# conservation-laws/ryujin

Hardware: AMD Instinct MI355X
Metric: MDoF-updates/s per Euler forward step; achieved HBM GB/s vs roofline (higher is better)
Workload: dtype f64; 1 GPU; 2D Euler Mach-3 forward-facing step, Q1, SSPRK33 stage sequence (BASELINE.json configs[1]); gridpoints_per_gpu=2498844, gridpoints_total=2498844, dofs_total=9995376, cells_per_unit=995, partition=x-slabs x1, equal gridpoint counts, develop_updates=600

## Files before the change

### include/ryujin_hip.h

```cpp
#ifndef RYUJIN_HIP_H
#define RYUJIN_HIP_H

#include <stddef.h>
#include <stdint.h>

#ifdef __cplusplus
extern "C" {
#endif

#define RYUJIN_OK 0
#define RYUJIN_WARN 1
#define RYUJIN_RESTART 2
#define RYUJIN_ERR_TAU (-1)
#define RYUJIN_ERR_ARG (-2)
#define RYUJIN_ERR_HIP (-3)
#define RYUJIN_ERR_COMM (-4)
#define RYUJIN_ERR_UNSUPPORTED (-5)

enum {
  RYUJIN_EQ_EULER = 0,
  RYUJIN_EQ_SHALLOW_WATER = 1,
  RYUJIN_EQ_EULER_AEOS = 2,
  RYUJIN_EQ_SCALAR_CONSERVATION = 3
};
// ... 66 lines not shown
  int sc_use_greedy_wavespeed;
  int sc_use_averaged_entropy;
  int sc_random_entropies;

  int system_scope_events;
  int debug_join_exchanges;
  int debug_bc_fold_max_slices;
  int debug_no_small_mesh_split;
  int debug_pij_storage;
  int debug_expensive_bounds_check;
  int debug_tile_map;
  int debug_band_stride;
  int debug_xcd_chunk;
  int debug_stencil_classes;
  int debug_next_tile_mask;
} ryujin_hip_params;

typedef struct ryujin_hip_offline {
  uint32_t n_export, n_internal, n_owned, n_relevant;
  uint32_t simd_length;
  const uint64_t *row_starts;
  const uint32_t *columns;
  const double *cij;
  const double *mij;
  const double *mi;
  const double *mi_inv;
  double measure_of_omega;

  uint32_t n_bdry;
  const uint32_t *b_i;
// ... 87 lines not shown

int ryujin_hip_set_cfl(ryujin_hip_ctx *ctx, double cfl);
int ryujin_hip_get_cfl(ryujin_hip_ctx *ctx, double *cfl);
int ryujin_hip_set_id_violation_strategy(ryujin_hip_ctx *ctx, int strategy);
int ryujin_hip_get_alpha(ryujin_hip_ctx *ctx, double *alpha );
int ryujin_hip_get_counters(ryujin_hip_ctx *ctx, unsigned *n_restarts, unsigned *n_warnings);
int ryujin_hip_limiter_statistics(ryujin_hip_ctx *ctx, double *limited_slice_fraction, int *pij_stored,
                                  double *stored_slice_fraction);
int ryujin_hip_layout_info(ryujin_hip_ctx *ctx, unsigned long long *n_tiles, unsigned long long *n_regular_tiles);
int ryujin_hip_chain_info(ryujin_hip_ctx *ctx, unsigned long long *n_chained_tiles,
                          unsigned long long *n_chained_entries);
int ryujin_hip_stencil_class_info(ryujin_hip_ctx *ctx, unsigned long long *n_uniform_slices,
                                  unsigned long long *n_classes, double *uniform_entry_fraction);
int ryujin_hip_next_tile_mask_info(ryujin_hip_ctx *ctx, int *active, unsigned long long *n_tiles,
                                   unsigned long long *n_named);
int ryujin_hip_tile_statistics(ryujin_hip_ctx *ctx, double *stored_fraction, double *read_fraction,
                               double *formed_by_step6_fraction);

int ryujin_hip_debug_fetch(ryujin_hip_ctx *ctx, int what, double *out, size_t n_doubles);
int ryujin_hip_debug_fill(ryujin_hip_ctx *ctx, int what, double value);
#define RYUJIN_DEBUG_PLAN_LENGTH 32
int ryujin_hip_debug_plan(ryujin_hip_ctx *ctx, int *out, int n);
int ryujin_hip_set_timers(ryujin_hip_ctx *ctx, int enable);
int ryujin_hip_get_timers(ryujin_hip_ctx *ctx, double ms[8]);
int ryujin_hip_get_timers_accum(ryujin_hip_ctx *ctx, double ms[8], unsigned *n_updates, int reset);
int ryujin_hip_synchronize(ryujin_hip_ctx *ctx);
int ryujin_hip_event_record(ryujin_hip_ctx *ctx, int which );
int ryujin_hip_event_elapsed_ms(ryujin_hip_ctx *ctx, double *ms);
int ryujin_hip_debug_layout(const ryujin_hip_offline *offline, uint64_t *ptr, uint32_t *col,
                            uint64_t *transposed, const double *data, uint32_t n_comp, double *out);
// ... 156 lines not shown
```

### ryujin_amd/capi.py

```python
from __future__ import annotations

import ctypes as C
import os

import numpy as np

from . import _build

c_double_p = C.POINTER(C.c_double)
c_u32_p = C.POINTER(C.c_uint32)
c_u64_p = C.POINTER(C.c_uint64)
c_u8_p = C.POINTER(C.c_uint8)
c_int_p = C.POINTER(C.c_int)

RYUJIN_OK, RYUJIN_WARN, RYUJIN_RESTART = 0, 1, 2
RYUJIN_ERR_TAU, RYUJIN_ERR_ARG, RYUJIN_ERR_HIP, RYUJIN_ERR_COMM, RYUJIN_ERR_UNSUPPORTED = -1, -2, -3, -4, -5
EQ_EULER, EQ_SHALLOW_WATER, EQ_EULER_AEOS, EQ_SCALAR_CONSERVATION = 0, 1, 2, 3
FLUX_BURGERS, FLUX_KPP, FLUX_POLYNOMIAL, FLUX_FUNCTION = 0, 1, 2, 3
EOS_POLYTROPIC_GAS, EOS_NOBLE_ABEL_STIFFENED_GAS, EOS_VAN_DER_WAALS, EOS_JONES_WILKINS_LEE = 0, 1, 2, 3
EOS_FUNCTION = 4
EOS_PRESSURE, EOS_SPECIFIC_INTERNAL_ENERGY, EOS_TEMPERATURE, EOS_SPEED_OF_SOUND = 0, 1, 2, 3
BC_DO_NOTHING, BC_PERIODIC, BC_SLIP, BC_NO_SLIP, BC_DIRICHLET, BC_DYNAMIC, BC_DIRICHLET_MOMENTUM = range(7)
IDV_WARN, IDV_RAISE_EXCEPTION = 0, 1
CUT_NONE, CUT_BOX, CUT_CYLINDER = 0, 1, 2
# ... 30 lines not shown
        ("riemann_newton_max_iterations", C.c_int), ("riemann_newton_tolerance", C.c_double),
        ("eos", C.c_int), ("compute_strict_bounds", C.c_int),
        ("eos_covolume_b", C.c_double), ("eos_q", C.c_double), ("eos_pinf", C.c_double),
        ("eos_vdw_a", C.c_double), ("eos_gas_constant_R", C.c_double),
        ("jwl_A", C.c_double), ("jwl_B", C.c_double), ("jwl_R1", C.c_double), ("jwl_R2", C.c_double),
        ("jwl_omega", C.c_double), ("jwl_rho_0", C.c_double), ("jwl_q_0", C.c_double),
        ("jwl_cv", C.c_double),
        ("sc_flux", C.c_int), ("sc_flux_polynomial", (C.c_double * 4) * 3),
        ("sc_derivative_approximation_delta", C.c_double), ("sc_use_greedy_wavespeed", C.c_int),
        ("sc_use_averaged_entropy", C.c_int), ("sc_random_entropies", C.c_int),
        ("system_scope_events", C.c_int), ("debug_join_exchanges", C.c_int),
        ("debug_bc_fold_max_slices", C.c_int), ("debug_no_small_mesh_split", C.c_int),
        ("debug_pij_storage", C.c_int), ("debug_expensive_bounds_check", C.c_int),
        ("debug_tile_map", C.c_int), ("debug_band_stride", C.c_int),
        ("debug_xcd_chunk", C.c_int), ("debug_stencil_classes", C.c_int),
        ("debug_next_tile_mask", C.c_int),
    ]


class Offline(C.Structure):
    _fields_ = [
        ("n_export", C.c_uint32), ("n_internal", C.c_uint32), ("n_owned", C.c_uint32),
        ("n_relevant", C.c_uint32), ("simd_length", C.c_uint32),
        ("row_starts", c_u64_p), ("columns", c_u32_p), ("cij", c_double_p), ("mij", c_double_p),
        ("mi", c_double_p), ("mi_inv", c_double_p), ("measure_of_omega", C.c_double),
        ("n_bdry", C.c_uint32), ("b_i", c_u32_p), ("b_normal", c_double_p), ("b_id", c_u8_p),
        ("n_pairs", C.c_uint32), ("p_i", c_u32_p), ("p_col", c_u32_p), ("p_j", c_u32_p),
        ("initial_precomputed", c_double_p),
        ("n_nbr", C.c_int), ("nbr_rank", c_int_p), ("send_off", c_u32_p), ("send_idx", c_u32_p),
        ("recv_off", c_u32_p), ("row_send_off", c_u32_p), ("row_send_row", c_u32_p),
        ("row_send_col", c_u32_p),
# ... 336 lines not shown
        lib.ryujin_offline_file_positions.argtypes = [C.c_void_p]
        lib.ryujin_offline_file_b_positions.restype = c_double_p
        lib.ryujin_offline_file_b_positions.argtypes = [C.c_void_p]
        _synth = lib
    return _synth



HIP_SYMBOLS = [
    "ryujin_hip_comm_unique_id", "ryujin_hip_comm_init", "ryujin_hip_comm_init_local",
    "ryujin_hip_comm_init_loopback",
    "ryujin_hip_comm_destroy", "ryujin_hip_comm_info", "ryujin_hip_exchange_info", "ryujin_hip_device_count",
    "ryujin_hip_time_step_fn", "ryujin_hip_debug_addresses",
    "ryujin_hip_host_register", "ryujin_hip_host_unregister", "ryujin_hip_state_download_owned",
    "ryujin_hip_state_download_prepared", "ryujin_hip_layout_info", "ryujin_hip_chain_info", "ryujin_hip_stencil_class_info", "ryujin_hip_tile_statistics",
    "ryujin_hip_next_tile_mask_info", "ryujin_hip_debug_fill",
    "ryujin_hip_default_params", "ryujin_hip_create", "ryujin_hip_destroy",
    "ryujin_hip_state_alloc", "ryujin_hip_state_free", "ryujin_hip_state_upload",
    "ryujin_hip_state_download", "ryujin_hip_state_download_precomputed", "ryujin_hip_state_integrals",
    "ryujin_hip_prepare_state_vector", "ryujin_hip_step", "ryujin_hip_sadd", "ryujin_hip_time_step", "ryujin_hip_time_step_n",
    "ryujin_hip_get_timers_accum",
    "ryujin_hip_set_cfl", "ryujin_hip_get_cfl", "ryujin_hip_set_id_violation_strategy",
    "ryujin_hip_get_alpha", "ryujin_hip_get_counters", "ryujin_hip_limiter_statistics", "ryujin_hip_debug_fetch", "ryujin_hip_debug_plan",
    "ryujin_hip_set_timers", "ryujin_hip_get_timers", "ryujin_hip_synchronize",
    "ryujin_hip_event_record", "ryujin_hip_event_elapsed_ms", "ryujin_hip_last_error",
    "ryujin_hip_version", "ryujin_hip_debug_layout", "ryujin_hip_debug_pow", "ryujin_hip_debug_function", "ryujin_hip_debug_rk_outcome",
    "ryujin_hip_postprocess_configure", "ryujin_hip_postprocess_compute", "ryujin_hip_postprocess_download",
    "ryujin_hip_postprocess_bounds",
    "ryujin_hip_quantities_add_manifold", "ryujin_hip_quantities_reset", "ryujin_hip_quantities_clear_statistics",
    "ryujin_hip_quantities_accumulate", "ryujin_hip_quantities_instantaneous", "ryujin_hip_quantities_time_averaged",
    "ryujin_hip_quantities_time_series",
# ... 70 lines not shown
        lib.ryujin_hip_time_step_n.argtypes = [vp, C.c_int, C.c_int, C.c_int, c_int_p, c_double_p, C.c_double,
                                               C.c_int, C.c_double, C.c_double, c_double_p]
        lib.ryujin_hip_time_step_fn.argtypes = [vp, C.c_int, C.c_int, C.c_int, c_int_p, C.c_double, DIRICHLET_FN,
                                                C.c_void_p, C.c_double, C.c_int, C.c_double, C.c_double, c_double_p]
        lib.ryujin_hip_device_count.argtypes = [c_int_p]
        lib.ryujin_hip_layout_info.argtypes = [vp, C.POINTER(C.c_ulonglong), C.POINTER(C.c_ulonglong)]
        lib.ryujin_hip_chain_info.argtypes = [vp, C.POINTER(C.c_ulonglong), C.POINTER(C.c_ulonglong)]
        if hasattr(lib, "ryujin_hip_stencil_class_info"):
            lib.ryujin_hip_stencil_class_info.argtypes = [vp, C.POINTER(C.c_ulonglong), C.POINTER(C.c_ulonglong),
                                                          C.POINTER(C.c_double)]
        if hasattr(lib, "ryujin_hip_debug_fill"):
            lib.ryujin_hip_debug_fill.argtypes = [vp, C.c_int, C.c_double]
        if hasattr(lib, "ryujin_hip_next_tile_mask_info"):
            lib.ryujin_hip_next_tile_mask_info.argtypes = [vp, c_int_p, C.POINTER(C.c_ulonglong),
                                                           C.POINTER(C.c_ulonglong)]
        lib.ryujin_hip_tile_statistics.argtypes = [vp, C.POINTER(C.c_double), C.POINTER(C.c_double), C.POINTER(C.c_double)]
        lib.ryujin_hip_host_register.argtypes = [vp, C.c_void_p, C.c_size_t]
        lib.ryujin_hip_host_unregister.argtypes = [vp, C.c_void_p]
        lib.ryujin_hip_state_download_owned.argtypes = [vp, C.c_int, c_double_p]
        lib.ryujin_hip_state_download_prepared.argtypes = [vp, C.c_int, c_double_p]
        lib.ryujin_hip_debug_addresses.argtypes = [vp, c_u64_p]
        lib.ryujin_hip_debug_plan.argtypes = [vp, c_int_p, C.c_int]
        lib.ryujin_hip_synchronize.argtypes = [vp]
        lib.ryujin_hip_event_record.argtypes = [vp, C.c_int]
        lib.ryujin_hip_event_elapsed_ms.argtypes = [vp, c_double_p]
        lib.ryujin_hip_version.restype = C.c_char_p
        lib.ryujin_hip_debug_layout.argtypes = [C.POINTER(Offline), c_u64_p, c_u32_p, c_u64_p,
                                                c_double_p, C.c_uint32, c_double_p]
        lib.ryujin_hip_debug_pow.argtypes = [C.c_int, c_double_p, c_double_p, c_double_p, C.c_size_t]
        lib.ryujin_hip_debug_rk_outcome.argtypes = [C.c_int, C.c_int, C.c_int]
# ... 52 lines not shown
```

### ryujin_amd/csrc/host_context.hpp

```cpp

#pragma once

#include <algorithm>
#include <atomic>
#include <cmath>
#include <cstdint>
#include <cstring>
#include <numeric>
#include <stdexcept>
#include <string>
#include <vector>

#include "host_layout.hpp"
#include "ryujin_hip.h"

namespace ryujin_hip
{
  struct HipError : std::runtime_error {
    int status;
    HipError(int status, const std::string &what)
        : std::runtime_error(what)
        , status(status)
    {
    }
// ... 45 lines not shown
      if (p.eos < RYUJIN_EOS_POLYTROPIC_GAS || p.eos > RYUJIN_EOS_FUNCTION)
        throw HipError(RYUJIN_ERR_UNSUPPORTED, "unknown equation of state");
      for (uint32_t b = 0; b < o.n_bdry; ++b)
        if (o.b_id[b] == RYUJIN_BC_DYNAMIC)
          throw HipError(RYUJIN_ERR_UNSUPPORTED,
                         "euler aeos: dynamic boundary conditions are not implemented in the reference");
    }
    if (p.equation == RYUJIN_EQ_SHALLOW_WATER && p.dim == 3)
      throw HipError(RYUJIN_ERR_UNSUPPORTED, "the shallow water equations are defined for dim 1 and 2");
    if (p.dim < 1 || p.dim > 3)
      throw HipError(RYUJIN_ERR_ARG, "dim must be 1, 2 or 3");
    if (p.limiter_iterations < 0 || p.limiter_iterations > 2)
      throw HipError(RYUJIN_ERR_ARG, "The number of limiter iterations must be between [0,2]");
    if (p.debug_stencil_classes > 1)
      throw HipError(RYUJIN_ERR_ARG, "debug_stencil_classes must be < 0 (off), 0 or 1 (classes without the table of norms)");
    if (p.debug_pij_storage > 2)
      throw HipError(RYUJIN_ERR_ARG, "debug_pij_storage must be < 0, 0, 1 or 2 (per-tile P_ij in 3-D was retired)");
    if (p.equation == RYUJIN_EQ_SCALAR_CONSERVATION && p.sc_flux == RYUJIN_FLUX_FUNCTION &&
        (!(p.sc_derivative_approximation_delta > 0.) || !std::isfinite(p.sc_derivative_approximation_delta)))
      throw HipError(RYUJIN_ERR_ARG, "flux: derivative approximation delta must be positive and finite");
    if (o.discontinuous_ansatz != 0) {
      if (p.equation == RYUJIN_EQ_SCALAR_CONSERVATION)
        throw HipError(RYUJIN_ERR_UNSUPPORTED,
                       "discontinuous ansatz with scalar conservation equations: the reference's Riemann solver is 0/0 "
                       "on the structural zeros of a dG stencil");
      if (!o.incidence || !o.mass_matrix_inverse)
        throw HipError(RYUJIN_ERR_ARG, "discontinuous ansatz without incidence / inverse mass matrix");
    }
    if (o.n_nbr > 0 && !have_comm)
      throw HipError(RYUJIN_ERR_COMM, "offline data has neighbour ranks but no communicator was given");
// ... 166 lines not shown
```

### ryujin_amd/csrc/kernels_euler.hpp

```cpp

#pragma once

#include <hip/hip_runtime.h>

#include <cfloat>
#include <cstdint>

#include "euler_device.hpp"

namespace ryujin_hip
{
  struct DeviceScalars;

  struct StencilClassEntry {
    double c[2];
    double m;
    int32_t delta;
    uint32_t pad;
  };
  static_assert(sizeof(StencilClassEntry) == 32, "four 64-bit words");

  struct StepBegin {
    DeviceScalars *scalars;
    double tau_max_in, tau_in;
// ... 79 lines not shown
#endif
#ifndef RYUJIN_OCC_LAST_3D
#define RYUJIN_OCC_LAST_3D 4
#endif
#ifndef RYUJIN_LAST_CHUNK_3D
#define RYUJIN_LAST_CHUNK_3D 3
#endif
#ifndef RYUJIN_LAST_CHUNK_2D
#define RYUJIN_LAST_CHUNK_2D 3
#endif
#ifndef RYUJIN_OCC_DIJ
#define RYUJIN_OCC_DIJ 2
#endif
#ifndef RYUJIN_OCC_LOW
#define RYUJIN_OCC_LOW 3
#endif
#ifndef RYUJIN_OCC_LOW_AEOS
#define RYUJIN_OCC_LOW_AEOS 2
#endif
#ifndef RYUJIN_OCC_PIJ
#define RYUJIN_OCC_PIJ 2
#endif
#ifndef RYUJIN_OCC_HO
#define RYUJIN_OCC_HO 2
#endif
#ifndef RYUJIN_PER_SLICE_MAX_LIMITED
#define RYUJIN_PER_SLICE_MAX_LIMITED 0.8
#endif

  constexpr int kBlock = 256;
// ... 884 lines not shown
          d = dij[pos];
        }
        d_sum -= d;
      }
    }
    double tau = DBL_MAX;
    if (row_active) {
      d_sum = fmin(d_sum, -1.e6 * DBL_MIN);
      dij[(uint64_t)r.base * 64 + r.lane] = d_sum;
      tau = cfl * M.mi[i] / (-2. * d_sum);
    }
    publish_tau_min(scalars, wave_min(tau), r.lane);
  }

  template <int MAXW>
  __global__ void __launch_bounds__(kBlock)
  k_dij_diag_unrolled(const DeviceMesh M, const uint32_t *__restrict__ lower_mask, const double cfl,
                      double *__restrict__ dij, DeviceScalars *__restrict__ scalars)
  {
    const RowCtx r = row_context(M);
    if (!r.valid)
      return;
    const bool row_active = r.len > 1;
    uint32_t mask = row_active ? lower_mask[r.row] : 0u;
    asm volatile("" : "+v"(mask));
    double d[MAXW];
#pragma unroll
    for (int c = 1; c < MAXW; ++c) {
      d[c] = 0.;
      if ((uint32_t)c < r.width) {
        const uint32_t pos = (r.base + c) * 64 + r.lane;
        const TileDesc t = tile_desc<(MAXW <= 9)>(M, (uint64_t)r.base + c);
        const uint32_t src = ((mask >> c) & 1u) ? tile_transposed(M, t, (uint64_t)r.base + c, r.lane) : pos;
// ... 6 lines not shown
      if ((uint32_t)c < r.width) {
        if ((mask >> c) & 1u)
          dij[(r.base + c) * 64 + r.lane] = d[c];
        if (row_active && (uint32_t)c < r.len)
          d_sum -= d[c];
      }
    }
    double tau = DBL_MAX;
    if (row_active) {
      d_sum = fmin(d_sum, -1.e6 * DBL_MIN);
      dij[(uint64_t)r.base * 64 + r.lane] = d_sum;
      tau = cfl * M.mi[r.row] / (-2. * d_sum);
    }
    publish_tau_min(scalars, wave_min(tau), r.lane);
  }

  RYUJIN_DEV double finalize_tau(DeviceScalars *scalars)
  {
    const double tau_max = __longlong_as_double((long long)scalars->tau_max_bits);
    const int use_device_tau = scalars->use_device_tau;
    const double tau_in = scalars->tau_in;
    const double tau = use_device_tau ? scalars->tau_rk : (tau_in == 0. ? tau_max : tau_in);
    if (blockIdx.x == 0 && threadIdx.x == 0) {
      const int invalid = (isnan(tau_max) || isinf(tau_max) || !(tau_max > 0.)) ? 1 : 0;
      const int stage = scalars->stage;
      scalars->tau_invalid = invalid;
      if (invalid && scalars->tau_invalid_accum < kStageCode - stage)
        scalars->tau_invalid_accum = kStageCode - stage;
      scalars->tau = tau;
      if (!use_device_tau)
// ... 35 lines not shown
  {
    const double denom = fmax(d_ij, 100. * DBL_MIN);
    return 1. / denom;
  }

  template <bool DG>
  RYUJIN_DEV double high_order_factor(const double alpha_i, const double alpha_j, const double *incidence,
                                      const uint64_t pos)
  {
    double factor = (alpha_i + alpha_j) * .5;
    if constexpr (DG)
      factor = fmax(factor, incidence[pos]);
    return factor;
  }

  template <int DIM, bool HAS_STAGES, bool STORE_P = true, bool DG = false>
  __global__ void __launch_bounds__(kBlock, (DIM == 3 && HAS_STAGES) ? 1 : ((DIM == 3 || HAS_STAGES || DG) ? 2 : RYUJIN_OCC_LOW))
  k_low_order(const EulerParams P, const DeviceMesh M, DeviceScalars *scalars,
              const double weight, const StageArgs<DIM> S, const double *__restrict__ U,
              const double *__restrict__ prec, const double *__restrict__ alpha,
              const double *__restrict__ dij, double *__restrict__ new_U, double *__restrict__ r_out,
              double *__restrict__ bounds, double *__restrict__ pij)
  {
    using E = Euler<DIM>;
    constexpr int K = E::K;
    const RowCtx r = row_context(M);
    if (!r.valid)
      return;
    const bool row_active = r.len > 1;
    const uint32_t i = row_active ? r.row : (r.row < M.n_owned ? r.row : M.n_owned - 1);
    const double tau = finalize_tau(scalars);

    double U_i[K], U_i_new[K], F_iH[K];
    load_state<K>(U, i, U_i);
#pragma unroll
    for (int q = 0; q < K; ++q) {
      U_i_new[q] = U_i[q];
// ... 28 lines not shown
        if constexpr (UNIFORM)
          return (uint32_t)((int32_t)i + class_delta(M, cls + (uint32_t)(colbase - r.base)));
        else
          return ld_stream(cols + (colbase * 64 + r.lane));
      };
      uint32_t j_n = column(r.base);
      uint32_t j_nn = r.width > 1 ? column((uint64_t)r.base + 1) : i;
      double c_n[DIM], U_n[K];
      if constexpr (UNIFORM)
        class_cij<DIM>(M, cls, c_n);
      else
        load_entry<DIM>(cij, r.base, r.lane, c_n);
      double d_n = dij[(uint64_t)r.base * 64 + r.lane];
      load_state<K>(U, j_n, U_n);
      double alpha_n = alpha[j_n];
      double s_n = prec[(size_t)j_n * 2 + 0];

      for (uint32_t c = 0; c < r.width; ++c) {
        const uint64_t colbase = (uint64_t)r.base + c;
        const bool active = UNIFORM ? row_active : (row_active && c < r.len);
        double c_ij[DIM], U_j[K];
        const uint32_t j = j_n;
#pragma unroll
        for (int d = 0; d < DIM; ++d)
          c_ij[d] = c_n[d];
#pragma unroll
        for (int q = 0; q < K; ++q)
          U_j[q] = U_n[q];
        const double d_ij = d_n, alpha_j = alpha_n, s_j = s_n;
        if (c + 1 < r.width) {
          j_n = j_nn;
          if constexpr (UNIFORM)
            class_cij<DIM>(M, cls + c + 1, c_n);
          else
            load_entry<DIM>(cij, colbase + 1, r.lane, c_n);
          d_n = dij[(colbase + 1) * 64 + r.lane];
          load_state<K>(U, j_n, U_n);
          alpha_n = alpha[j_n];
          s_n = prec[(size_t)j_n * 2 + 0];
          j_nn = (c + 2 < r.width) ? column(colbase + 2) : i;
        }

        if (!active)
          continue;

        const double d_ijH = d_ij * high_order_factor<DG>(alpha_i, alpha_j, M.incidence, colbase * 64 + r.lane);
        double scaled_c_ij[DIM];
        const double inverse_denom = inverse_regularized(d_ij);
#pragma unroll
        for (int d = 0; d < DIM; ++d)
          scaled_c_ij[d] = c_ij[d] * inverse_denom;

        double f_j[K][DIM];
        E::flux(P, U_j, f_j);
// ... 25 lines not shown
          const double dU = U_j[q] - U_i[q];
          U_i_new[q] += tau * m_i_inv * d_ij * dU;
          F_iH[q] += d_ijH * dU;
          P_ij[q] += (d_ijH - d_ij) * dU;
        }

        {
          const double rho_i = U_i[0], rho_j = U_j[0];
          double dm_c = (U_i[1] - U_j[1]) * scaled_c_ij[0];
#pragma unroll
          for (int d = 1; d < DIM; ++d)
            dm_c += (U_i[1 + d] - U_j[1 + d]) * scaled_c_ij[d];
          const double rho_ij_bar = 0.5 * (rho_i + rho_j + dm_c) + 0.;
          rho_min = fmin(rho_min, rho_ij_bar);
          rho_max = fmax(rho_max, rho_ij_bar);
          s_min = fmin(s_min, s_j);
          rho_relaxation_numerator += 1. * (rho_i + rho_j);
          rho_relaxation_denominator += 1.;
          double U_avg[K];
#pragma unroll
          for (int q = 0; q < K; ++q)
            U_avg[q] = (U_i[q] + U_j[q]) * .5;
          const double s_interp = c == 0 ? s_j : E::specific_entropy(P, U_avg);
          s_interp_max = fmax(s_interp_max, s_interp);
        }

#pragma unroll
        for (int q = 0; q < K; ++q) {
          F_iH[q] += weight * flux_ij[q];
          P_ij[q] += weight * flux_ij[q];
        }

        if constexpr (HAS_STAGES) {
          for (int s = 0; s < S.stages; ++s) {
            double U_iHs[K], U_jHs[K];
            load_state<K>(S.U[s], i, U_iHs);
            load_state<K>(S.U[s], j, U_jHs);
            double f_iHs[K][DIM], f_jHs[K][DIM];
            E::flux(P, U_iHs, f_iHs);
// ... 16 lines not shown
    dispatch_uniform<kClasses>(cls, column_loop);

    if (!row_active)
      return;

    store_state<K>(new_U, i, U_i_new);
    store_state<K>(r_out, i, F_iH);

    const double hd_i = m_i * M.measure_of_omega_inverse;
    const double r_i = relaxation_radius<DIM>(hd_i) * P.lim_relaxation_factor;
    const double rho_relaxation =
        fabs(rho_relaxation_numerator) / (fabs(rho_relaxation_denominator) + DBL_EPSILON);
    const double relaxation = (2. * P.lim_relaxation_factor) * rho_relaxation;
    const double rho_min_r = fmax((1. - r_i) * rho_min, rho_min - relaxation);
    const double rho_max_r = fmin((1. + r_i) * rho_max, rho_max + relaxation);
    const double entropy_relaxation = P.lim_relaxation_factor * (s_interp_max - s_min);
    const double s_min_r = fmax((1. - r_i) * s_min, s_min - entropy_relaxation);

    const size_t stride = M.bounds_stride;
    bounds[i] = rho_min_r;
    bounds[stride + i] = rho_max_r;
    bounds[2 * stride + i] = s_min_r;
  }

  template <int NB, unsigned MAX_MASK>
  __global__ void __launch_bounds__(kBlock)
  k_bounds_combine_minmax(const DeviceMesh M, const double *__restrict__ in, double *__restrict__ out)
  {
    const RowCtx r = row_context(M);
    if (!r.valid)
      return;
    const bool row_active = r.len > 1;
    const uint32_t i = row_active ? r.row : (r.row < M.n_owned ? r.row : M.n_owned - 1);
    const size_t stride = M.bounds_stride;
    double b[NB];
#pragma unroll
    for (int q = 0; q < NB; ++q)
// ... 165 lines not shown
```

### ryujin_amd/csrc/ryujin_hip.hip

```cpp

#include <hip/hip_runtime.h>
#include <rccl/rccl.h>

#include <algorithm>
#include <atomic>
#include <cmath>
#include <cstddef>
#include <cstdlib>
#include <cstring>
#include <condition_variable>
#include <limits>
#include <memory>
#include <mutex>
#include <numeric>
#include <string>
#include <type_traits>
#include <vector>

#include "ryujin_hip.h"

#ifndef RYUJIN_XCD_CHUNK_3D
#define RYUJIN_XCD_CHUNK_3D 8
#endif

// ... 1274 lines not shown
{
  StepPlanInput in;
  in.equation = is_euler_v<E> ? PlanEquation::euler
                              : (is_aeos_v<E> ? PlanEquation::euler_aeos
                                              : (is_scalar_v<E> ? PlanEquation::scalar : PlanEquation::shallow_water));
  in.dim = E::DIMENSION;
  in.fusable_precompute = E::kFusablePrecompute;
  in.stages = stages;
  in.limiter_iterations = params.limiter_iterations;
  in.dg = dg;
  in.max_row_len = L.max_row_len;
  in.n_slices = L.n_slices;
  in.n_export_slices = exch.n_nbr != 0 ? n_export_slices : 0u;
  in.debug_pij_storage = params.debug_pij_storage;
  in.debug_next_tile_mask = params.debug_next_tile_mask;
  in.checked = params.debug_expensive_bounds_check != 0;
  in.limited_fraction = limited_fraction;
  in.per_slice_max_limited = (double)RYUJIN_PER_SLICE_MAX_LIMITED;
  in.resident_waves_step5 = resident_waves_step5;
  in.resident_waves_step6 = resident_waves_step6;
  in.bc_fold_max_slices = bc_fold_max_slices;
  in.pending_precompute = pending_precompute;
  in.riemann_newton_max_iterations = eparams.riemann_newton_max_iterations;
  in.rarefaction_power = eparams.rarefaction_power;
  in.friction = swparams.manning != 0.;
  return in;
}

template <typename E>
void ryujin_hip_ctx::step2_dij_alpha(const StepPlan &plan, const State &old)
// ... 71 lines not shown
      if (flux_interpreted_pairs())
        hipLaunchKernelGGL(k_dij_boundary_sc_function<DIM>, dim3(grid_for(n_pairs, kFluxFunctionBlock)),
                           dim3(kFluxFunctionBlock), 0, stream, eparams, d_flux_function.ptr, n_pairs, d_p_i.ptr,
                           d_p_j.ptr, d_p_pos.ptr, d_p_cji.ptr, old.U.ptr, old.prec.ptr, d_dij.ptr);
      else
        hipLaunchKernelGGL(k_dij_boundary_sc<DIM>, dim3(grid_for(n_pairs)), block, 0, stream, eparams,
                           n_pairs, d_p_i.ptr, d_p_j.ptr, d_p_pos.ptr, d_p_cji.ptr, old.U.ptr,
                           old.prec.ptr, d_dij.ptr);
    }
    else
      hipLaunchKernelGGL(k_dij_boundary<E>, dim3(grid_for(n_pairs)), block, 0, stream, eparams,
                         n_pairs, d_p_i.ptr, d_p_j.ptr, d_p_pos.ptr, d_p_cji.ptr, old.U.ptr, d_dij.ptr);
  }
  sweep([&](const DeviceMesh &mm, dim3 grid) {
    auto unrolled = [&](auto width) {
      hipLaunchKernelGGL(k_dij_diag_unrolled<decltype(width)::value>, grid, block, 0, launch_stream, mm,
                         d_lower_mask.ptr, params.cfl, d_dij.ptr, d_scalars.ptr);
    };
    if (plan.diag_width == 3)
      unrolled(std::integral_constant<int, 3>{});
    else if (plan.diag_width == 9)
      unrolled(std::integral_constant<int, 9>{});
    else if (plan.diag_width == 27)
      unrolled(std::integral_constant<int, 27>{});
    else
      hipLaunchKernelGGL(k_dij_diag, grid, block, 0, launch_stream, mm, params.cfl, d_dij.ptr,
                         d_scalars.ptr);
  });
  if (!(deferred && rk_stage > 0))
    allreduce_scalar(&d_scalars.ptr->tau_max_bits, 0);
  if (want_tau_early && deferred && rk_stage == 0) {
// ... 46 lines not shown
          });
        });
      }
    }
    auto launch4 = [&](auto has_stages, auto stores_p, auto dg_) {
      constexpr bool HS = decltype(has_stages)::value, SP = decltype(stores_p)::value, DG = decltype(dg_)::value;
      if constexpr (is_euler_v<E>)
        launch(k_low_order<DIM, HS, SP, DG>);
      else if constexpr (is_aeos_v<E>)
        launch(k_low_order_aeos<DIM, HS, SP, DG>);
      else if constexpr (is_scalar_v<E>)
        launch(k_low_order_sc<DIM, HS, DG>);
      else
        launch(k_low_order_sw<DIM, HS, DG>, d_Z.ptr);
    };
    if (!plan.step4_stores_p)
      launch4(std::false_type{}, std::false_type{}, std::false_type{});
    else
      with_bool(plan.step4_has_stages, [&](auto has_stages) {
        with_bool(plan.dg, [&](auto dg_) { launch4(has_stages, std::true_type{}, dg_); });
      });
  });
  if (plan.checked)
    sweep([&](const DeviceMesh &mm, dim3 grid) {
      hipLaunchKernelGGL(k_check_admissible<E>, grid, block, 0, launch_stream, eparams, mm, d_scalars.ptr,
                         (const double *)nw.U.ptr);
    });
  exchange_vector(d_r.ptr, KP, true);
  if (plan.dg && plan.step5 != StepPlan::Step5::none) {
    for (int b = 0; b < NB; ++b)
// ... 871 lines not shown
  p->sc_derivative_approximation_delta = 1.e-10;
  p->sc_use_greedy_wavespeed = 0;
  p->sc_use_averaged_entropy = 0;
  p->sc_random_entropies = 0;
  p->system_scope_events = 0;
  p->debug_join_exchanges = 0;
  p->debug_bc_fold_max_slices = 0;
  p->debug_no_small_mesh_split = 0;
  p->debug_pij_storage = 0;
  p->debug_expensive_bounds_check = 0;
  p->debug_tile_map = 0;
  p->debug_band_stride = 0;
  p->debug_xcd_chunk = 0;
  p->debug_stencil_classes = 0;
  p->debug_next_tile_mask = 0;
  if (const char *e = std::getenv("RYUJIN_XCD_CHUNK"))
    p->debug_xcd_chunk = std::atoi(e);
  if (const char *e = std::getenv("RYUJIN_BAND_STRIDE"))
    p->debug_band_stride = std::atoi(e);
}

int ryujin_hip_comm_unique_id(char id[RYUJIN_HIP_UNIQUE_ID_BYTES])
{
  return guarded([&]() {
    static_assert(sizeof(ncclUniqueId) <= RYUJIN_HIP_UNIQUE_ID_BYTES, "unique id size");
    ncclUniqueId uid;
    NCCL_CHECK(ncclGetUniqueId(&uid));
    std::memset(id, 0, RYUJIN_HIP_UNIQUE_ID_BYTES);
    std::memcpy(id, &uid, sizeof(uid));
    return RYUJIN_OK;
// ... 544 lines not shown
                          hipMemcpyDeviceToHost));
    }
    unsigned long long tiles = 0, named = 0;
    for (uint32_t s = 0; s < L.n_slices; ++s) {
      const uint32_t width = L.slice_off[s + 1] - L.slice_off[s];
      const uint32_t off_diagonal = width > 1 ? width - 1 : 0u;
      tiles += off_diagonal;
      named += on ? (unsigned long long)__builtin_popcount(words[s] & ~1u) : off_diagonal;
    }
    if (active)
      *active = on ? 1 : 0;
    if (n_tiles)
      *n_tiles = tiles;
    if (n_named)
      *n_named = named;
    return RYUJIN_OK;
  });
}

int ryujin_hip_debug_plan(ryujin_hip_ctx *ctx, int *out, int n)
{
  return guarded([&]() {
    if (!ctx || (n > 0 && !out) || n < 0)
      throw HipError(RYUJIN_ERR_ARG, "null context or output");
    const StepPlan &p = ctx->last_plan;
    const auto &log = ctx->last_launches;
    int v[RYUJIN_DEBUG_PLAN_LENGTH] = {(int)p.step2,
                                       p.step2_split,
                                       p.fast_riemann,
                                       p.diag_width,
// ... 1846 lines not shown
```

### ryujin_amd/csrc/step_plan.hpp

```cpp
#ifndef RYUJIN_HIP_STEP_PLAN_HPP
#define RYUJIN_HIP_STEP_PLAN_HPP

#include <algorithm>
#include <cstdint>

namespace ryujin_hip
{
  enum class PlanEquation { euler, euler_aeos, scalar, shallow_water };

  constexpr uint32_t kPlanWavesPerBlock = 4;

  constexpr int q1_stencil_width(const int dim) { return dim == 1 ? 3 : (dim == 2 ? 9 : 27); }

  struct StepPlanInput {
    PlanEquation equation = PlanEquation::euler;
    int dim = 1;
    bool fusable_precompute = false;
    int stages = 0, limiter_iterations = 2;
    bool dg = false;
    uint32_t max_row_len = 0, n_slices = 0;
    uint32_t n_export_slices = 0;
    int debug_pij_storage = 0;
    int debug_next_tile_mask = 0;
    bool checked = false;
    double limited_fraction = 1.;
    double per_slice_max_limited = 1.;
    uint32_t resident_waves_step5 = 0, resident_waves_step6 = 0, bc_fold_max_slices = 0;
    bool pending_precompute = false;
    int riemann_newton_max_iterations = 0, rarefaction_power = 0;
    bool friction = false;
  };

  struct StepPlan {
    int dim = 1;
    uint32_t resident_waves_step5 = 0, resident_waves_step6 = 0;
    enum class Step2 {
      alpha_then_dij,
      dij_alpha_sc,
      records,
      dij_alpha
    } step2 = Step2::dij_alpha;
    bool step2_split = false;
    bool fast_riemann = false;
    int diag_width = 0;
    bool step4_single_walk = false, step4_has_stages = false, step4_friction = false, step4_stores_p = true;
    bool dg = false;
    enum class Step5 { none, stage0_per_tile, stage0_per_slice, stage0_groups, recompute, pij_lij } step5 = Step5::none;
    uint32_t step5_groups = 1;
    bool wide = false;
    bool has_V = false;
    int pij_stored = 1;
    bool tiles_predicted_from_history = false;
    enum class Step6 { none, per_slice, cached, high_order } step6 = Step6::none;
    bool step6_flags = false;
    enum class Step7 { none, last_cached, high_order } step7 = Step7::none;
    bool next_tile_mask = false;
    bool next_tiles_elided = false;
    bool fuse_precompute = false;
    bool checked = false;
    const char *unsupported = nullptr, *violated = nullptr;
// ... 22 lines not shown
  inline const char *next_tile_mask_violated(const StepPlan &p, const uint32_t n_slices, const uint32_t n_export_slices)
  {
    if (!p.next_tile_mask)
      return p.next_tiles_elided ? "step plan: zeros are elided under the tile mask only" : nullptr;
    if (p.step6 != StepPlan::Step6::cached || p.dim > 2)
      return "step plan: the tile mask needs the single-launch cached step 6, dim <= 2";
    if (some_launch_shares_slices(p, n_slices, n_export_slices))
      return "step plan: the tile mask needs one wave per slice in every launch of step 6";
    if (p.step7 != StepPlan::Step7::last_cached)
      return "step plan: the tile mask needs the cached step 7";
    if (p.checked)
      return "step plan: the checked kernels read all of l_ij";
    return nullptr;
  }

  inline StepPlan plan_step(const StepPlanInput &in)
  {
    const bool is_euler = in.equation == PlanEquation::euler, is_aeos = in.equation == PlanEquation::euler_aeos;
    const bool is_scalar = in.equation == PlanEquation::scalar, is_sw = in.equation == PlanEquation::shallow_water;
    const int n_iterations = in.limiter_iterations;
    const uint32_t q1_width = (uint32_t)q1_stencil_width(in.dim);
    StepPlan p;
    p.dim = in.dim;
    p.resident_waves_step5 = in.resident_waves_step5;
    p.resident_waves_step6 = in.resident_waves_step6;
    p.checked = in.checked;
    p.dg = in.dg;
    p.wide = in.max_row_len > 64;

    p.fast_riemann = is_euler && in.riemann_newton_max_iterations == 0 && in.rarefaction_power > 0;
// ... 11 lines not shown
      p.step2 = StepPlan::Step2::dij_alpha;
    p.step2_split = p.step2 == StepPlan::Step2::alpha_then_dij || p.step2 == StepPlan::Step2::dij_alpha_sc;

    p.diag_width = in.max_row_len <= 3 ? 3 : (in.max_row_len <= 9 ? 9 : (in.max_row_len <= 27 ? 27 : 0));

    const bool recompute_p =
        is_euler && in.dim <= 2 && in.stages == 0 && n_iterations != 0 && !in.dg && in.max_row_len <= 64;
    const bool stage0_pij =
        (is_euler || is_aeos) && in.stages == 0 && n_iterations != 0 && !in.dg && in.max_row_len <= q1_width;

    p.step4_single_walk = is_sw && !in.dg && in.max_row_len <= (uint32_t)(in.dim == 1 ? 3 : 9);
    p.step4_has_stages = in.stages != 0;
    p.step4_friction = is_sw && in.friction;
    p.step4_stores_p = !(recompute_p || stage0_pij);

    const uint32_t step5_groups = std::min<uint32_t>(
        4u, in.resident_waves_step5 /
                std::max<uint32_t>(1u, (in.n_slices + kPlanWavesPerBlock - 1) / kPlanWavesPerBlock * kPlanWavesPerBlock));
    const int storage = in.debug_pij_storage;
    const bool selective = stage0_pij && n_iterations == 2 && step5_groups < 2 && storage >= 0 && !in.checked;
    const bool tile_store = in.dim <= 2 && selective && storage != 1;
    const bool per_slice =
        selective && !tile_store && (storage != 0 || in.limited_fraction <= in.per_slice_max_limited);
    p.pij_stored = per_slice ? 2 : (tile_store ? 3 : 1);
    p.tiles_predicted_from_history = tile_store && storage == 0;

    const bool two_passes = n_iterations == 2;
    if (n_iterations == 0)
      p.step5 = StepPlan::Step5::none;
    else if (stage0_pij) {
// ... 22 lines not shown
    p.next_tiles_elided = p.next_tile_mask && in.debug_next_tile_mask == 0;

    p.fuse_precompute = in.fusable_precompute && in.pending_precompute && n_iterations != 0 &&
                        in.n_slices > in.bc_fold_max_slices && cached;

    if (p.per_tile() && !(p.has_V && p.step5 == StepPlan::Step5::stage0_per_tile && p.step5_groups == 1 && in.dim <= 2))
      p.violated = "step plan: P_ij per tile needs V_i, one wave per slice and dim <= 2";
    else if (p.per_slice() && !(p.has_V && p.step5 == StepPlan::Step5::stage0_per_slice))
      p.violated = "step plan: P_ij per slice needs V_i";
    else if (p.wide && p.step5 != StepPlan::Step5::none && p.step5 != StepPlan::Step5::pij_lij)
      p.violated = "step plan: rows of more than 64 entries need k_pij_lij<WIDE> in step 5";
    else if (p.checked && p.pij_stored != 1)
      p.violated = "step plan: the checked kernels read all of P_ij";
    else if (const char *v = next_tile_mask_violated(p, in.n_slices, in.n_export_slices))
      p.violated = v;
    return p;
  }
}

#endif
```

### ryujin_amd/module.py

```python
from __future__ import annotations

import ctypes as C

import numpy as np

from . import capi


class Restart(Exception):
    """Mirror of ryujin::Restart (source/hyperbolic_module.h:49-57)."""


class TauError(RuntimeError):
    """tau_max is NaN/inf/<=0 (AssertThrow at hyperbolic_module.template.h:573-576)."""


class StateVector:

    def __init__(self, module: "HyperbolicModule"):
        self.module = module
        h = C.c_int(-1)
        module._check(module._f("state_alloc")(module._ctx, C.byref(h)))
        self.handle = h.value

# ... 559 lines not shown
        return dict(n_tiles=n.value, n_regular_tiles=r.value,
                    regular_tile_fraction=(r.value / n.value if n.value else 0.0),
                    n_chained_tiles=ch.value, chained_tile_fraction=(ch.value / n.value if n.value else 0.0),
                    chained_entry_fraction=(ce.value / (64.0 * n.value) if n.value else 0.0))

    def stencil_class_info(self) -> dict:
        n, k, f = C.c_ulonglong(0), C.c_ulonglong(0), C.c_double(0.0)
        self._check(self._lib.ryujin_hip_stencil_class_info(self._ctx, C.byref(n), C.byref(k), C.byref(f)))
        return dict(n_uniform_slices=n.value, n_classes=k.value, uniform_entry_fraction=f.value)

    def next_tile_mask_info(self) -> dict:
        a, n, k = C.c_int(0), C.c_ulonglong(0), C.c_ulonglong(0)
        self._check(self._lib.ryujin_hip_next_tile_mask_info(self._ctx, C.byref(a), C.byref(n), C.byref(k)))
        return dict(active=bool(a.value), n_tiles=n.value, n_named=k.value)

    PLAN_STEP2 = ("alpha_then_dij", "dij_alpha_sc", "records", "dij_alpha")
    PLAN_STEP5 = ("none", "stage0_per_tile", "stage0_per_slice", "stage0_groups", "recompute", "pij_lij")
    PLAN_STEP6 = ("none", "per_slice", "cached", "high_order")
    PLAN_STEP7 = ("none", "last_cached", "high_order")

    def last_plan(self) -> dict:
        n = 32
        v = (C.c_int * n)()
        rc = self._lib.ryujin_hip_debug_plan(self._ctx, v, n)
        if rc != n:
            self._check(rc if rc < 0 else capi.RYUJIN_ERR_ARG)
        flags = ("step2_split", "fast_riemann", None, "step4_single_walk", "step4_has_stages", "step4_friction",
                 "step4_stores_p", "dg", None, None, "wide", "has_V", None, "tiles_predicted_from_history", None,
                 "step6_flags", None, "fuse_precompute", "checked")
        out = dict(step2=self.PLAN_STEP2[v[0]], diag_width=v[3], step5=self.PLAN_STEP5[v[9]], step5_groups=v[10],
# ... 232 lines not shown
```

Before: 9287 MDoF-updates/s.

## Move entropy bound computation from low-order step into step-3 diagonal kernel

Adds a step-3 kernel that computes dij's diagonal and also walks each row to form the relaxed specific-entropy lower bound, writing it into the bounds array. A matching step-4 low-order kernel then skips reading neighbour entropies and computing averaged-state entropies, which lowers its register pressure and permits a higher occupancy bound. It applies only to Euler without stages, DG or stored P_ij, with unrolled width 3 or 9. The step-3 kernel now reads the full neighbour state, so those loads may be duplicated across the two kernels.

```diff
diff --git a/include/ryujin_hip.h b/include/ryujin_hip.h
--- a/include/ryujin_hip.h
+++ b/include/ryujin_hip.h
@@ -104,6 +104,7 @@
   int debug_xcd_chunk;
   int debug_stencil_classes;
   int debug_next_tile_mask;
+  int debug_entropy_in_step3;
 } ryujin_hip_params;
 
 typedef struct ryujin_hip_offline {
@@ -221,6 +222,7 @@
                                   unsigned long long *n_classes, double *uniform_entry_fraction);
 int ryujin_hip_next_tile_mask_info(ryujin_hip_ctx *ctx, int *active, unsigned long long *n_tiles,
                                    unsigned long long *n_named);
+int ryujin_hip_entropy_bound_info(ryujin_hip_ctx *ctx, int *active);
 int ryujin_hip_tile_statistics(ryujin_hip_ctx *ctx, double *stored_fraction, double *read_fraction,
                                double *formed_by_step6_fraction);
 
diff --git a/ryujin_amd/capi.py b/ryujin_amd/capi.py
--- a/ryujin_amd/capi.py
+++ b/ryujin_amd/capi.py
@@ -68,7 +68,7 @@
         ("debug_pij_storage", C.c_int), ("debug_expensive_bounds_check", C.c_int),
         ("debug_tile_map", C.c_int), ("debug_band_stride", C.c_int),
         ("debug_xcd_chunk", C.c_int), ("debug_stencil_classes", C.c_int),
-        ("debug_next_tile_mask", C.c_int),
+        ("debug_next_tile_mask", C.c_int), ("debug_entropy_in_step3", C.c_int),
     ]
 
 
@@ -435,7 +435,7 @@
     "ryujin_hip_time_step_fn", "ryujin_hip_debug_addresses",
     "ryujin_hip_host_register", "ryujin_hip_host_unregister", "ryujin_hip_state_download_owned",
     "ryujin_hip_state_download_prepared", "ryujin_hip_layout_info", "ryujin_hip_chain_info", "ryujin_hip_stencil_class_info", "ryujin_hip_tile_statistics",
-    "ryujin_hip_next_tile_mask_info", "ryujin_hip_debug_fill",
+    "ryujin_hip_next_tile_mask_info", "ryujin_hip_entropy_bound_info", "ryujin_hip_debug_fill",
     "ryujin_hip_default_params", "ryujin_hip_create", "ryujin_hip_destroy",
     "ryujin_hip_state_alloc", "ryujin_hip_state_free", "ryujin_hip_state_upload",
     "ryujin_hip_state_download", "ryujin_hip_state_download_precomputed", "ryujin_hip_state_integrals",
@@ -536,6 +536,8 @@
         if hasattr(lib, "ryujin_hip_next_tile_mask_info"):
             lib.ryujin_hip_next_tile_mask_info.argtypes = [vp, c_int_p, C.POINTER(C.c_ulonglong),
                                                            C.POINTER(C.c_ulonglong)]
+        if hasattr(lib, "ryujin_hip_entropy_bound_info"):
+            lib.ryujin_hip_entropy_bound_info.argtypes = [vp, c_int_p]
         lib.ryujin_hip_tile_statistics.argtypes = [vp, C.POINTER(C.c_double), C.POINTER(C.c_double), C.POINTER(C.c_double)]
         lib.ryujin_hip_host_register.argtypes = [vp, C.c_void_p, C.c_size_t]
         lib.ryujin_hip_host_unregister.argtypes = [vp, C.c_void_p]
diff --git a/ryujin_amd/csrc/host_context.hpp b/ryujin_amd/csrc/host_context.hpp
--- a/ryujin_amd/csrc/host_context.hpp
+++ b/ryujin_amd/csrc/host_context.hpp
@@ -83,6 +83,8 @@
       throw HipError(RYUJIN_ERR_ARG, "The number of limiter iterations must be between [0,2]");
     if (p.debug_stencil_classes > 1)
       throw HipError(RYUJIN_ERR_ARG, "debug_stencil_classes must be < 0 (off), 0 or 1 (classes without the table of norms)");
+    if (p.debug_entropy_in_step3 > 0)
+      throw HipError(RYUJIN_ERR_ARG, "debug_entropy_in_step3 must be < 0 (off) or 0");
     if (p.debug_pij_storage > 2)
       throw HipError(RYUJIN_ERR_ARG, "debug_pij_storage must be < 0, 0, 1 or 2 (per-tile P_ij in 3-D was retired)");
     if (p.equation == RYUJIN_EQ_SCALAR_CONSERVATION && p.sc_flux == RYUJIN_FLUX_FUNCTION &&
diff --git a/ryujin_amd/csrc/kernels_euler.hpp b/ryujin_amd/csrc/kernels_euler.hpp
--- a/ryujin_amd/csrc/kernels_euler.hpp
+++ b/ryujin_amd/csrc/kernels_euler.hpp
@@ -117,6 +117,15 @@
 #endif
 #ifndef RYUJIN_OCC_LOW
 #define RYUJIN_OCC_LOW 3
+#endif
+#ifndef RYUJIN_OCC_LOW_ENTROPY_GIVEN
+#define RYUJIN_OCC_LOW_ENTROPY_GIVEN 4
+#endif
+#ifndef RYUJIN_OCC_DIAG_ENTROPY
+#define RYUJIN_OCC_DIAG_ENTROPY 5
+#endif
+#ifndef RYUJIN_OCC_LOW_ENTROPY_GIVEN_3D
+#define RYUJIN_OCC_LOW_ENTROPY_GIVEN_3D 3
 #endif
 #ifndef RYUJIN_OCC_LOW_AEOS
 #define RYUJIN_OCC_LOW_AEOS 2
@@ -1031,9 +1040,8 @@
   }
 
   template <int MAXW>
-  __global__ void __launch_bounds__(kBlock)
-  k_dij_diag_unrolled(const DeviceMesh M, const uint32_t *__restrict__ lower_mask, const double cfl,
-                      double *__restrict__ dij, DeviceScalars *__restrict__ scalars)
+  RYUJIN_DEV void dij_diag_unrolled_sweep(const DeviceMesh M, const uint32_t *lower_mask, const double cfl,
+                                          double *dij, DeviceScalars *scalars)
   {
     const RowCtx r = row_context(M);
     if (!r.valid)
@@ -1070,6 +1078,15 @@
     }
     publish_tau_min(scalars, wave_min(tau), r.lane);
   }
+
+  template <int MAXW>
+  __global__ void __launch_bounds__(kBlock)
+  k_dij_diag_unrolled(const DeviceMesh M, const uint32_t *__restrict__ lower_mask, const double cfl,
+                      double *__restrict__ dij, DeviceScalars *__restrict__ scalars)
+  {
+    dij_diag_unrolled_sweep<MAXW>(M, lower_mask, cfl, dij, scalars);
+  }
+
 
   RYUJIN_DEV double finalize_tau(DeviceScalars *scalars)
   {
@@ -1135,13 +1152,19 @@
     return factor;
   }
 
-  template <int DIM, bool HAS_STAGES, bool STORE_P = true, bool DG = false>
-  __global__ void __launch_bounds__(kBlock, (DIM == 3 && HAS_STAGES) ? 1 : ((DIM == 3 || HAS_STAGES || DG) ? 2 : RYUJIN_OCC_LOW))
-  k_low_order(const EulerParams P, const DeviceMesh M, DeviceScalars *scalars,
-              const double weight, const StageArgs<DIM> S, const double *__restrict__ U,
-              const double *__restrict__ prec, const double *__restrict__ alpha,
-              const double *__restrict__ dij, double *__restrict__ new_U, double *__restrict__ r_out,
-              double *__restrict__ bounds, double *__restrict__ pij)
+
+  RYUJIN_DEV double relaxed_entropy_bound(const EulerParams &P, const double r_i, const double s_min,
+                                          const double s_interp_max)
+  {
+    const double entropy_relaxation = P.lim_relaxation_factor * (s_interp_max - s_min);
+    return fmax((1. - r_i) * s_min, s_min - entropy_relaxation);
+  }
+
+  template <int DIM, bool HAS_STAGES, bool STORE_P, bool DG, bool ENTROPY_GIVEN>
+  RYUJIN_DEV void low_order_sweep(const EulerParams P, const DeviceMesh M, DeviceScalars *scalars,
+                                  const double weight, const StageArgs<DIM> S, const double *U, const double *prec,
+                                  const double *alpha, const double *dij, double *new_U, double *r_out,
+                                  double *bounds, double *pij)
   {
     using E = Euler<DIM>;
     constexpr int K = E::K;
@@ -1200,7 +1223,7 @@
       double d_n = dij[(uint64_t)r.base * 64 + r.lane];
       load_state<K>(U, j_n, U_n);
       double alpha_n = alpha[j_n];
-      double s_n = prec[(size_t)j_n * 2 + 0];
+      double s_n = ENTROPY_GIVEN ? 0. : prec[(size_t)j_n * 2 + 0];
 
       for (uint32_t c = 0; c < r.width; ++c) {
         const uint64_t colbase = (uint64_t)r.base + c;
@@ -1223,7 +1246,8 @@
           d_n = dij[(colbase + 1) * 64 + r.lane];
           load_state<K>(U, j_n, U_n);
           alpha_n = alpha[j_n];
-          s_n = prec[(size_t)j_n * 2 + 0];
+          if constexpr (!ENTROPY_GIVEN)
+            s_n = prec[(size_t)j_n * 2 + 0];
           j_nn = (c + 2 < r.width) ? column(colbase + 2) : i;
         }
 
@@ -1279,15 +1303,18 @@
           const double rho_ij_bar = 0.5 * (rho_i + rho_j + dm_c) + 0.;
           rho_min = fmin(rho_min, rho_ij_bar);
           rho_max = fmax(rho_max, rho_ij_bar);
-          s_min = fmin(s_min, s_j);
+          if constexpr (!ENTROPY_GIVEN)
+            s_min = fmin(s_min, s_j);
           rho_relaxation_numerator += 1. * (rho_i + rho_j);
           rho_relaxation_denominator += 1.;
-          double U_avg[K];
-#pragma unroll
-          for (int q = 0; q < K; ++q)
-            U_avg[q] = (U_i[q] + U_j[q]) * .5;
-          const double s_interp = c == 0 ? s_j : E::specific_entropy(P, U_avg);
-          s_interp_max = fmax(s_interp_max, s_interp);
+          if constexpr (!ENTROPY_GIVEN) {
+            double U_avg[K];
+#pragma unroll
+            for (int q = 0; q < K; ++q)
+              U_avg[q] = (U_i[q] + U_j[q]) * .5;
+            const double s_interp = c == 0 ? s_j : E::specific_entropy(P, U_avg);
+            s_interp_max = fmax(s_interp_max, s_interp);
+          }
         }
 
 #pragma unroll
@@ -1334,13 +1361,109 @@
     const double relaxation = (2. * P.lim_relaxation_factor) * rho_relaxation;
     const double rho_min_r = fmax((1. - r_i) * rho_min, rho_min - relaxation);
     const double rho_max_r = fmin((1. + r_i) * rho_max, rho_max + relaxation);
-    const double entropy_relaxation = P.lim_relaxation_factor * (s_interp_max - s_min);
-    const double s_min_r = fmax((1. - r_i) * s_min, s_min - entropy_relaxation);
 
     const size_t stride = M.bounds_stride;
     bounds[i] = rho_min_r;
     bounds[stride + i] = rho_max_r;
-    bounds[2 * stride + i] = s_min_r;
+    if constexpr (!ENTROPY_GIVEN)
+      bounds[2 * stride + i] = relaxed_entropy_bound(P, r_i, s_min, s_interp_max);
+  }
+
+  template <int DIM, bool HAS_STAGES, bool STORE_P = true, bool DG = false>
+  __global__ void __launch_bounds__(kBlock, (DIM == 3 && HAS_STAGES) ? 1 : ((DIM == 3 || HAS_STAGES || DG) ? 2 : RYUJIN_OCC_LOW))
+  k_low_order(const EulerParams P, const DeviceMesh M, DeviceScalars *scalars,
+              const double weight, const StageArgs<DIM> S, const double *__restrict__ U,
+              const double *__restrict__ prec, const double *__restrict__ alpha,
+              const double *__restrict__ dij, double *__restrict__ new_U, double *__restrict__ r_out,
+              double *__restrict__ bounds, double *__restrict__ pij)
+  {
+    low_order_sweep<DIM, HAS_STAGES, STORE_P, DG, false>(P, M, scalars, weight, S, U, prec, alpha, dij, new_U, r_out,
+                                                         bounds, pij);
+  }
+
+  template <int DIM>
+  __global__ void __launch_bounds__(kBlock, DIM == 3 ? RYUJIN_OCC_LOW_ENTROPY_GIVEN_3D : RYUJIN_OCC_LOW_ENTROPY_GIVEN)
+  k_low_order_entropy_given(const EulerParams P, const DeviceMesh M, DeviceScalars *scalars, const double weight,
+                            const StageArgs<DIM> S, const double *__restrict__ U, const double *__restrict__ prec,
+                            const double *__restrict__ alpha, const double *__restrict__ dij,
+                            double *__restrict__ new_U, double *__restrict__ r_out, double *__restrict__ bounds,
+                            double *__restrict__ pij)
+  {
+    low_order_sweep<DIM, false, false, false, true>(P, M, scalars, weight, S, U, prec, alpha, dij, new_U, r_out,
+                                                    bounds, pij);
+  }
+
+
+  template <int DIM, int MAXW>
+  __global__ void __launch_bounds__(kBlock, DIM == 3 ? 4 : RYUJIN_OCC_DIAG_ENTROPY)
+  k_dij_diag_entropy(const DeviceMesh M, const uint32_t *__restrict__ lower_mask, const double cfl,
+                     double *__restrict__ dij, DeviceScalars *__restrict__ scalars, const EulerParams P,
+                     const double *__restrict__ U, const double *__restrict__ prec, double *__restrict__ bounds)
+  {
+    using E = Euler<DIM>;
+    constexpr int K = E::K;
+    dij_diag_unrolled_sweep<MAXW>(M, lower_mask, cfl, dij, scalars);
+    const RowCtx r = row_context(M);
+    if (!r.valid)
+      return;
+
+    const bool row_active = r.len > 1;
+    const uint32_t i = row_active ? r.row : (r.row < M.n_owned ? r.row : M.n_owned - 1);
+    double U_i[K];
+    load_state<K>(U, i, U_i);
+    const double s_i = prec[(size_t)i * 2 + 0];
+    double s_min = fmin(DBL_MAX, s_i), s_interp_max = fmax(0., s_i);
+
+    const uint32_t *__restrict__ cols = M.cols;
+    constexpr bool kClasses = stencil_classes_pay<DIM>();
+    const uint32_t cls = kClasses ? slice_stencil_class(M, r.slice) : kStencilClassNone;
+    auto column_loop = [&](auto uniform_) __attribute__((always_inline)) {
+      constexpr bool UNIFORM = decltype(uniform_)::value;
+      if (r.width < 2)
+        return;
+      auto column = [&](const uint64_t colbase) -> uint32_t {
+        if constexpr (UNIFORM)
+          return (uint32_t)((int32_t)i + class_delta(M, cls + (uint32_t)(colbase - r.base)));
+        else
+          return ld_stream(cols + (colbase * 64 + r.lane));
+      };
+      uint32_t j_n = column((uint64_t)r.base + 1);
+      uint32_t j_nn = r.width > 2 ? column((uint64_t)r.base + 2) : i;
+      double U_n[K];
+      load_state<K>(U, j_n, U_n);
+      double s_n = prec[(size_t)j_n * 2 + 0];
+
+      for (uint32_t c = 1; c < r.width; ++c) {
+        const uint64_t colbase = (uint64_t)r.base + c;
+        const bool active = UNIFORM ? row_active : (row_active && c < r.len);
+        double U_j[K];
+#pragma unroll
+        for (int q = 0; q < K; ++q)
+          U_j[q] = U_n[q];
+        const double s_j = s_n;
+        if (c + 1 < r.width) {
+          j_n = j_nn;
+          load_state<K>(U, j_n, U_n);
+          s_n = prec[(size_t)j_n * 2 + 0];
+          j_nn = (c + 2 < r.width) ? column(colbase + 2) : i;
+        }
+        if (!active)
+          continue;
+        s_min = fmin(s_min, s_j);
+        double U_avg[K];
+#pragma unroll
+        for (int q = 0; q < K; ++q)
+          U_avg[q] = (U_i[q] + U_j[q]) * .5;
+        s_interp_max = fmax(s_interp_max, E::specific_entropy(P, U_avg));
+      }
+    };
+    dispatch_uniform<kClasses>(cls, column_loop);
+
+    if (!row_active)
+      return;
+    const double hd_i = M.mi[i] * M.measure_of_omega_inverse;
+    const double r_i = relaxation_radius<DIM>(hd_i) * P.lim_relaxation_factor;
+    bounds[2 * M.bounds_stride + i] = relaxed_entropy_bound(P, r_i, s_min, s_interp_max);
   }
 
   template <int NB, unsigned MAX_MASK>
diff --git a/ryujin_amd/csrc/ryujin_hip.hip b/ryujin_amd/csrc/ryujin_hip.hip
--- a/ryujin_amd/csrc/ryujin_hip.hip
+++ b/ryujin_amd/csrc/ryujin_hip.hip
@@ -1312,6 +1312,7 @@
   in.n_export_slices = exch.n_nbr != 0 ? n_export_slices : 0u;
   in.debug_pij_storage = params.debug_pij_storage;
   in.debug_next_tile_mask = params.debug_next_tile_mask;
+  in.debug_entropy_in_step3 = params.debug_entropy_in_step3;
   in.checked = params.debug_expensive_bounds_check != 0;
   in.limited_fraction = limited_fraction;
   in.per_slice_max_limited = (double)RYUJIN_PER_SLICE_MAX_LIMITED;
@@ -1413,7 +1414,16 @@
   }
   sweep([&](const DeviceMesh &mm, dim3 grid) {
     auto unrolled = [&](auto width) {
-      hipLaunchKernelGGL(k_dij_diag_unrolled<decltype(width)::value>, grid, block, 0, launch_stream, mm,
+      constexpr int W = decltype(width)::value;
+      if constexpr (is_euler_v<E> && (W <= 9 || DIM == 3)) {
+        if (plan.entropy_bound_in_step3) {
+          hipLaunchKernelGGL((k_dij_diag_entropy<DIM, W>), grid, block, 0, launch_stream, mm, d_lower_mask.ptr,
+                             params.cfl, d_dij.ptr, d_scalars.ptr, eparams, (const double *)old.U.ptr,
+                             (const double *)old.prec.ptr, d_bounds.ptr);
+          return;
+        }
+      }
+      hipLaunchKernelGGL(k_dij_diag_unrolled<W>, grid, block, 0, launch_stream, mm,
                          d_lower_mask.ptr, params.cfl, d_dij.ptr, d_scalars.ptr);
     };
     if (plan.diag_width == 3)
@@ -1490,6 +1500,10 @@
       else
         launch(k_low_order_sw<DIM, HS, DG>, d_Z.ptr);
     };
+    if constexpr (is_euler_v<E>) {
+      if (plan.entropy_bound_in_step3)
+        return launch(k_low_order_entropy_given<DIM>);
+    }
     if (!plan.step4_stores_p)
       launch4(std::false_type{}, std::false_type{}, std::false_type{});
     else
@@ -2391,6 +2405,7 @@
   p->debug_xcd_chunk = 0;
   p->debug_stencil_classes = 0;
   p->debug_next_tile_mask = 0;
+  p->debug_entropy_in_step3 = 0;
   if (const char *e = std::getenv("RYUJIN_XCD_CHUNK"))
     p->debug_xcd_chunk = std::atoi(e);
   if (const char *e = std::getenv("RYUJIN_BAND_STRIDE"))
@@ -2965,6 +2980,17 @@
       *n_tiles = tiles;
     if (n_named)
       *n_named = named;
+    return RYUJIN_OK;
+  });
+}
+
+int ryujin_hip_entropy_bound_info(ryujin_hip_ctx *ctx, int *active)
+{
+  return guarded([&]() {
+    if (!ctx)
+      throw HipError(RYUJIN_ERR_ARG, "null context");
+    if (active)
+      *active = ctx->last_plan.entropy_bound_in_step3 ? 1 : 0;
     return RYUJIN_OK;
   });
 }
diff --git a/ryujin_amd/csrc/step_plan.hpp b/ryujin_amd/csrc/step_plan.hpp
--- a/ryujin_amd/csrc/step_plan.hpp
+++ b/ryujin_amd/csrc/step_plan.hpp
@@ -22,6 +22,7 @@
     uint32_t n_export_slices = 0;
     int debug_pij_storage = 0;
     int debug_next_tile_mask = 0;
+    int debug_entropy_in_step3 = 0;
     bool checked = false;
     double limited_fraction = 1.;
     double per_slice_max_limited = 1.;
@@ -44,6 +45,7 @@
     bool fast_riemann = false;
     int diag_width = 0;
     bool step4_single_walk = false, step4_has_stages = false, step4_friction = false, step4_stores_p = true;
+    bool entropy_bound_in_step3 = false;
     bool dg = false;
     enum class Step5 { none, stage0_per_tile, stage0_per_slice, stage0_groups, recompute, pij_lij } step5 = Step5::none;
     uint32_t step5_groups = 1;
@@ -96,6 +98,19 @@
     return nullptr;
   }
 
+  inline const char *entropy_bound_violated(const StepPlan &p, const bool is_euler)
+  {
+    if (!p.entropy_bound_in_step3)
+      return nullptr;
+    if (!is_euler)
+      return "step plan: the entropy bound from step 3 is Euler's";
+    if (p.diag_width != 3 && p.diag_width != 9)
+      return "step plan: the entropy bound from step 3 needs the unrolled step 3 of 3 or 9 columns";
+    if (p.step4_single_walk || p.step4_has_stages || p.step4_stores_p || p.dg)
+      return "step plan: the entropy bound from step 3 needs the plain step 4";
+    return nullptr;
+  }
+
   inline StepPlan plan_step(const StepPlanInput &in)
   {
     const bool is_euler = in.equation == PlanEquation::euler, is_aeos = in.equation == PlanEquation::euler_aeos;
@@ -137,6 +152,9 @@
     p.step4_friction = is_sw && in.friction;
     p.step4_stores_p = !(recompute_p || stage0_pij);
 
+    p.entropy_bound_in_step3 = in.debug_entropy_in_step3 >= 0 && is_euler && in.stages == 0 && !in.dg &&
+                               n_iterations != 0 && (p.diag_width == 3 || p.diag_width == 9) && !p.step4_stores_p;
+
     const uint32_t step5_groups = std::min<uint32_t>(
         4u, in.resident_waves_step5 /
                 std::max<uint32_t>(1u, (in.n_slices + kPlanWavesPerBlock - 1) / kPlanWavesPerBlock * kPlanWavesPerBlock));
@@ -189,6 +207,8 @@
       p.violated = "step plan: the checked kernels read all of P_ij";
     else if (const char *v = next_tile_mask_violated(p, in.n_slices, in.n_export_slices))
       p.violated = v;
+    else if (const char *v = entropy_bound_violated(p, is_euler))
+      p.violated = v;
     return p;
   }
 }
diff --git a/ryujin_amd/module.py b/ryujin_amd/module.py
--- a/ryujin_amd/module.py
+++ b/ryujin_amd/module.py
@@ -597,6 +597,11 @@
         self._check(self._lib.ryujin_hip_next_tile_mask_info(self._ctx, C.byref(a), C.byref(n), C.byref(k)))
         return dict(active=bool(a.value), n_tiles=n.value, n_named=k.value)
 
+    def entropy_bound_info(self) -> dict:
+        a = C.c_int(0)
+        self._check(self._lib.ryujin_hip_entropy_bound_info(self._ctx, C.byref(a)))
+        return dict(active=bool(a.value))
+
     PLAN_STEP2 = ("alpha_then_dij", "dij_alpha_sc", "records", "dij_alpha")
     PLAN_STEP5 = ("none", "stage0_per_tile", "stage0_per_slice", "stage0_groups", "recompute", "pij_lij")
     PLAN_STEP6 = ("none", "per_slice", "cached", "high_order")
```

Result: slower. 8952 MDoF-updates/s (-3.6%).
